# crowsonkb/k-diffusion

Measured on AMD Instinct MI355X. Metric: images/sec, 256x256 image_transformer_v2, 50-step DPM++2M (whole job), higher is better.
Workload: dtype f32

## Files before the change

include/kdiff_hip.h:

```cpp
#ifndef KDIFF_HIP_H
#define KDIFF_HIP_H

#ifdef __cplusplus
extern "C" {
#endif

#define KD_OK 0
#define KD_EINVAL (-1)
#define KD_ELAUNCH (-2)

int kd_version(void);
const char* kd_last_error(void);
int kd_set_option(const char* name, int value);
int kd_get_option(const char* name, int dflt);

enum { KD_A_PLAIN = 0, KD_A_MERGE2x2 = 1, KD_A_PATCH_NCHW = 2 };
enum { KD_PREC_EXACT = 0, KD_PREC_SPLIT3 = 1,
       KD_PREC_BF16 = 2  };
enum { KD_EPI_STORE = 0, KD_EPI_RESIDUAL = 1, KD_EPI_GEGLU = 2, KD_EPI_SPLIT_LERP = 3, KD_EPI_UNPATCH_NCHW = 4,
       KD_EPI_QKV = 5  };

typedef struct {
  int M, N, K;
  int a_mode, epi;
// ... 21 lines not shown
  int qkv_packed;
  const float* rope_pos;
  const float* rope_freq;
  int a_split, c_split;
  const void* A_lo;
  void* C_lo;
  int per_row;
} KdGemm;

int kd_gemm_f32(const KdGemm* desc, void* stream);

int kd_gemm_bf16(const KdGemm* desc, void* stream);
long long kd_packed_weight_bytes_bf16(int N, int K, int geglu);
int kd_pack_weight_bf16(const float* W, void* out, int N, int K, int geglu, void* stream);

typedef struct KdFfn {
  const void* x;
  void* out;
  const float* scale;
  int scale_stride, rows_per_sample;
  float eps;
  const void* Wp_up;
  const void* Wp_down;
  int M, K, d_ff;
  const void* attn;
  const void* Wp_out;
} KdFfn;
int kd_ffn_bf16_supported(int M, int K, int d_ff);
int kd_ffn_bf16(const KdFfn* desc, void* stream);
int kd_ffn_f32_supported(int M, int K, int d_ff);
int kd_ffn_f32(const KdFfn* desc, void* stream);
int kd_attn_ffn_f32_supported(int batch, int H, int W, int nh, int ks, int K, int d_ff);
int kd_attn_ffn_f32(const float* qkv, const KdFfn* desc, int batch, int H, int W, int nh, int ks, void* stream);

long long kd_packed_weight_bytes(int N, int K, int geglu);
int kd_pack_weight_bf16x3(const float* W, void* out, int N, int K, int geglu, void* stream);

int kd_norm_split_f32(const float* x, const float* scale, int scale_stride, int rows_per_sample, void* hi, void* lo, int M, int K,
                      float eps, void* stream);

int kd_rmsnorm_f32(const float* x, const float* scale, float* y, int rows, int d, float eps, void* stream);

int kd_fourier_sigma_f32(const float* sigma, const float* weight, float* ff, int batch, int half, void* stream);
int kd_fourier_f32(const float* in, const float* weight, float* ff, int batch, int in_dim, int half, void* stream);
int kd_cond_sum_f32(float* out, const float* a, const float* b, int b_rows, const float* emb,
                    const long long* ids, const float* c, int batch, int d, void* stream);

int kd_qk_prep_f32(float* qkv, const float* scale_h, const float* cos_t, const float* sin_t,
                   int batch, int tokens_per_sample, int nh, float eps, void* stream);

int kd_attn_global_f32(const float* qkv, float* out, int batch, int T, int nh,
                       int prep, const float* scale_h, const float* cos_t, const float* sin_t, float eps,
                       int precision, void* stream);

int kd_attn_window_f32(const float* qkv, float* out, int batch, int H, int W, int nh, int ws, int shift,
                       int prep, const float* scale_h, const float* cos_t, const float* sin_t, float eps,
                       int precision, void* stream);

int kd_attn_na2d_f32(const float* qkv, float* out, int batch, int H, int W, int nh, int ks,
                     int prep, const float* scale_h, const float* cos_t, const float* sin_t, float eps,
                     int precision, void* stream);

int kd_attn_global_bf16(const void* qkv, void* out, int batch, int T, int nh, void* stream);
int kd_attn_window_bf16(const void* qkv, void* out, int batch, int H, int W, int nh, int ws, int shift, void* stream);
int kd_attn_na2d_bf16(const void* qkv, void* out, int batch, int H, int W, int nh, int ks, void* stream);

// ... 142 lines not shown

int kd_pack_conv_x3(const float* w, void* out, int c_out, int c_in, int ks, void* stream);
int kd_conv2d_x3(const float* x, int ldx, const void* wp, const float* bias, const float* res, int ldr, float* y, int ldy, int batch, int H, int W,
                 int c_in, int c_out, int ks, void* stream);
int kd_conv2d_x3_stacked(const float* x, int ldx, const void* wp, const float* bias, const float* res, int ldr, float* y, int ldy, int batch, int H,
                         int W, int c_in, int c_out, int ks, int bias_batch, void* stream);
int kd_groupnorm_stats_f32(const float* x, int ldx, float* stats, int batch, int hw, int chan, int groups, float eps, void* stream);
int kd_groupnorm_stats_jvp_f32(const float* x, int ldx, const float* x_dot, int ldxd, float* stats, float* jstats, int batch, int hw, int chan,
                               int groups, float eps, void* stream);
int kd_adagn_apply_f32(const float* x, int ldx, const float* stats, const float* wb, int wb_stride, float* y, int ldy, int batch, int hw, int chan,
                       int groups, int gelu, void* stream);
int kd_adagn_apply_jvp_f32(const float* x, int ldx, const float* x_dot, int ldxd, const float* stats, const float* jstats, const float* wb,
                           int wb_stride, float* y, int ldy, float* y_dot, int ldyd, int batch, int hw, int chan, int groups, int gelu, void* stream);
int kd_down2_f32(const float* x, int ldx, float* y, int ldy, int batch, int H, int W, int chan, void* stream);
int kd_up2_f32(const float* x, int ldx, float* y, int ldy, int batch, int H, int W, int chan, void* stream);
int kd_unet_in_f32(const float* img, const float* w, const float* bias, const float* sigma, float sigma_data, float* y, int ldy, int batch, int hw,
                   int c_img, int chan, void* stream);
int kd_unet_out_f32(const float* x, int ldx, const float* w, const float* bias, const float* img, const float* sigma, float sigma_data, float* out,
                    int batch, int hw, int c_img, int chan, void* stream);
int kd_cond_mlp_f32(const float* x, const float* w, const float* bias, const float* add, float* y, int rows, int n_out, int k_in, int gelu,
                    void* stream);

int kd_to_uint8(const float* x, unsigned char* y, long long n, void* stream);

int kd_prof_enable(int on);
int kd_prof_count(void);
int kd_prof_get(int i, char* name, int name_cap, float* ms, double* flops, double* bytes);
int kd_prof_reset(void);
int kd_prof_clock_buffer(void* dev_ptr);

enum { KD_OP_GEMM_F32 = 0, KD_OP_GEMM_BF16 = 1, KD_OP_FFN_F32 = 2, KD_OP_FFN_BF16 = 3,
       KD_OP_ATTN_GLOBAL_F32 = 4, KD_OP_ATTN_WINDOW_F32 = 5, KD_OP_ATTN_NA2D_F32 = 6,
       KD_OP_ATTN_GLOBAL_BF16 = 7, KD_OP_ATTN_WINDOW_BF16 = 8, KD_OP_ATTN_NA2D_BF16 = 9, KD_OP_NORM_SPLIT_F32 = 10,
       KD_OP_ATTN_BLOCK_BF16 = 11, KD_OP_PROJ_BLOCK_BF16 = 12, KD_OP_GEMM_MX8 = 13, KD_OP_ATTN_FFN_F32 = 14 };
typedef struct {
  int op;
  float f;
  const void* p[5];
  int i[8];
} KdCall;
int kd_run_list(const KdCall* calls, int n, void* stream, int* failed);

#ifdef __cplusplus
}
#endif
#endif
```

k-diffusion_amd/_native.py:

```python
import ctypes as C
import os

_HERE = os.path.dirname(os.path.abspath(__file__))
LIB_PATH = os.environ.get("KDIFF_HIP_LIB") or os.path.join(_HERE, "csrc", "libkdiff_hip.so")

A_PLAIN, A_MERGE2x2, A_PATCH_NCHW = 0, 1, 2
EPI_STORE, EPI_RESIDUAL, EPI_GEGLU, EPI_SPLIT_LERP, EPI_UNPATCH_NCHW, EPI_QKV = 0, 1, 2, 3, 4, 5
PREC_EXACT, PREC_SPLIT3, PREC_BF16 = 0, 1, 2
PC_ONE, PC_SKIP, PC_OUT, PC_IN = 0, 1, 2, 3
WG_PLAIN, WG_MERGE2x2, WG_PATCH_NCHW = 0, 1, 2
LW_KARRAS, LW_SOFT_MIN_SNR, LW_SNR, LW_GIVEN = 0, 1, 2, 3
PREC_FP8 = 3
_MODES = {"exact": PREC_EXACT, "split3": PREC_SPLIT3, "bf16": PREC_BF16, "fp8": PREC_FP8}


def default_precision():
    mode = os.environ.get("KDIFF_GEMM", "split3").lower()
    if mode not in _MODES:
        raise ValueError(f"KDIFF_GEMM={mode!r}: expected one of {sorted(_MODES)}")
    return _MODES[mode]


def kernel_precision():
    p = default_precision()
# ... 39 lines not shown

class KdMtTensor(C.Structure):
    _fields_ = [("p", C.c_void_p), ("g", C.c_void_p), ("m", C.c_void_p), ("v", C.c_void_p), ("ema", C.c_void_p),
                ("n", C.c_longlong), ("group", C.c_int), ("reserved", C.c_int)]


class KdAdamGroup(C.Structure):
    _fields_ = [("lr", C.c_double), ("wd", C.c_double), ("beta1", C.c_double), ("beta2", C.c_double), ("eps", C.c_double),
                ("bc1", C.c_double), ("bc2", C.c_double)]


MT_CHUNK = 8192
(DENSITY_LOGNORMAL, DENSITY_LOGLOGISTIC, DENSITY_LOGUNIFORM, DENSITY_V_DIFFUSION, DENSITY_COSINE_INTERPOLATED,
 DENSITY_SPLIT_LOGNORMAL) = range(6)

_vp, _i, _f, _ll, _d = C.c_void_p, C.c_int, C.c_float, C.c_longlong, C.c_double
_u, _ull = C.c_uint, C.c_ulonglong

SIGNATURES = {
    "kd_version": [],
    "kd_last_error": [],
    "kd_set_option": [C.c_char_p, _i],
    "kd_get_option": [C.c_char_p, _i],
    "kd_gemm_f32": [C.POINTER(KdGemm), _vp],
    "kd_gemm_bf16": [C.POINTER(KdGemm), _vp],
    "kd_packed_weight_bytes_bf16": [_i, _i, _i],
    "kd_pack_weight_bf16": [_vp, _vp, _i, _i, _i, _vp],
    "kd_ffn_bf16_supported": [_i, _i, _i],
    "kd_ffn_bf16": [_vp, _vp],
    "kd_ffn_f32_supported": [_i, _i, _i],
    "kd_ffn_f32": [_vp, _vp],
    "kd_attn_ffn_f32_supported": [_i, _i, _i, _i, _i, _i, _i],
    "kd_attn_ffn_f32": [_vp, _vp, _i, _i, _i, _i, _i, _vp],
    "kd_attn_global_bf16": [_vp, _vp, _i, _i, _i, _vp],
    "kd_attn_window_bf16": [_vp, _vp, _i, _i, _i, _i, _i, _i, _vp],
    "kd_attn_na2d_bf16": [_vp, _vp, _i, _i, _i, _i, _i, _vp],
    "kd_attn_block_bf16_supported": [_i, _i, _i],
    "kd_attn_block_bf16": [C.POINTER(KdGemm), _vp],
    "kd_proj_block_bf16_supported": [_i, _i, _i, _i],
    "kd_proj_block_bf16": [C.POINTER(KdGemm), _vp],
    "kd_packed_weight_bytes_mx8": [_i, _i, _i],
    "kd_pack_weight_mx8": [_vp, _vp, _i, _i, _i, _vp],
    "kd_gemm_mx8_supported": [_i, _i, _i, _i, _i],
    "kd_gemm_mx8": [C.POINTER(KdGemm), _vp],
    "kd_packed_weight_bytes": [_i, _i, _i],
    "kd_pack_weight_bf16x3": [_vp, _vp, _i, _i, _i, _vp],
    "kd_rmsnorm_f32": [_vp, _vp, _vp, _i, _i, _f, _vp],
    "kd_fourier_sigma_f32": [_vp, _vp, _vp, _i, _i, _vp],
    "kd_fourier_f32": [_vp, _vp, _vp, _i, _i, _i, _vp],
    "kd_cond_sum_f32": [_vp, _vp, _vp, _i, _vp, _vp, _vp, _i, _i, _vp],
    "kd_qk_prep_f32": [_vp, _vp, _vp, _vp, _i, _i, _i, _f, _vp],
    "kd_attn_global_f32": [_vp, _vp, _i, _i, _i, _i, _vp, _vp, _vp, _f, _i, _vp],
    "kd_attn_window_f32": [_vp, _vp, _i, _i, _i, _i, _i, _i, _i, _vp, _vp, _vp, _f, _i, _vp],
    "kd_attn_na2d_f32": [_vp, _vp, _i, _i, _i, _i, _i, _i, _vp, _vp, _vp, _f, _i, _vp],
    "kd_sampler_step_f32": [_i, _vp, _vp, _vp, _vp, _vp, _f, _f, _f, _f, _ll, _vp],
    "kd_precond_in_f32": [_vp, _vp, _vp, _f, _i, _ll, _vp],
    "kd_precond_out_f32": [_vp, _vp, _vp, _vp, _f, _i, _ll, _vp],
    "kd_rows_affine_f32": [_vp, _vp, _vp, _vp, _vp, _i, _ll, _vp],
    "kd_sigma_to_t_f32": [_vp, _vp, _vp, _i, _i, _i, _vp],
    "kd_t_to_sigma_f32": [_vp, _vp, _vp, _i, _i, _vp],
    "kd_dpm_eps_f32": [_vp, _vp, _vp, _f, _ll, _vp],
    "kd_dpm_combine_f32": [_vp, _vp, _vp, _vp, _f, _f, _ll, _vp],
    "kd_dpm_error_partials": [],
    "kd_dpm_error_f32": [_vp, _vp, _vp, _f, _f, _ll, _vp, _vp],
    "kd_brownian_f32": [_vp, _vp, _i, _ll, _d, _d, _d, _d, _f, _i, _vp],
    "kd_brownian_cached_f32": [_vp, _vp, _vp, _i, _i, _vp, _i, _ll, _d, _d, _d, _d, _f, _i, _vp],
# ... 42 lines not shown
    "kd_row_rrms_f32": [_vp, _vp, _ll, _i, _f, _vp],
    "kd_colsum_f32": [_vp, _vp, _vp, _vp, _ll, _i, _ll, _i, _vp, _vp, _vp],
    "kd_attn_scale_grad_f32": [_vp, _vp, _i, _i, _vp, _vp],
    "kd_class_emb_grad_f32": [_vp, _vp, _i, _i, _i, _i, _vp, _vp],
    "kd_loss_prep_f32": [_vp, _vp, _vp, _f, _vp, _vp, _i, _ll, _vp],
    "kd_loss_f32": [_vp, _vp, _vp, _vp, _f, _i, _vp, _vp, _i, _ll, _vp],
    "kd_loss_vjp_f32": [_vp, _vp, _vp, _vp, _f, _i, _vp, _vp, _vp, _i, _ll, _vp],
    "kd_mmd_poly_f32": [_vp, _ll, _ll, _vp, _ll, _ll, _i, _i, _i, _vp, _f, _i, _vp, _vp],
    "kd_poly_kernel_f32": [_vp, _ll, _ll, _vp, _ll, _ll, _i, _i, _i, _vp, _vp],
    "kd_mmd_mats_f32": [_vp, _vp, _vp, _ll, _ll, _i, _vp, _vp, _vp],
    "kd_jacobi_sweep_f64": [_vp, _vp, _i, _i, _d, _vp, _vp, _vp],
    "kd_sym_lower_f64": [_vp, _i, _vp, _vp, _i, _i, _d, _vp],
    "kd_row_sqrt_norm_f64": [_vp, _ll, _i, _vp, _vp],
    "kd_gemm_tn_f64": [_vp, _vp, _vp, _i, _i, _i, _i, _vp, _vp, _vp],
    "kd_center_f32": [_vp, _vp, _ll, _i, _vp, _vp, _vp],
    "kd_transpose_f64": [_vp, _vp, _i, _i, _vp],
    "kd_sqrtm_vjp_div_f64": [_vp, _vp, _i, _i, _vp, _vp],
    "kd_f32_to_f64": [_vp, _vp, _ll, _vp],
    "kd_fid_finish_f32": [_vp, _vp, _vp, _vp, _vp, _i, _vp, _vp],
    "kd_mt_sqnorm_f32": [_vp, _vp, _i, _f, _vp, _vp, _vp],
    "kd_mt_adamw_ema_f32": [_vp, _vp, _i, _vp, _i, _vp, _d, _i, _i, _vp],
    "kd_mt_lerp_f32": [_vp, _vp, _i, _d, _vp],
    "kd_sigma_density_f32": [_i, _vp, _i, _vp, _vp, _i, _ll, _i, _i, _i, _vp, _vp],
    "kd_prof_enable": [_i],
    "kd_prof_count": [],
    "kd_prof_get": [_i, C.c_char_p, _i, C.POINTER(C.c_float), C.POINTER(C.c_double), C.POINTER(C.c_double)],
    "kd_prof_reset": [],
    "kd_prof_clock_buffer": [_vp],
    "kd_run_list": [C.POINTER(KdCall), _i, _vp, C.POINTER(C.c_int)],
}

RUN_LIST_OPS = {"kd_gemm_f32": 0, "kd_gemm_bf16": 1, "kd_ffn_f32": 2, "kd_ffn_bf16": 3, "kd_attn_global_f32": 4, "kd_attn_window_f32": 5,
                "kd_attn_na2d_f32": 6, "kd_attn_global_bf16": 7, "kd_attn_window_bf16": 8, "kd_attn_na2d_bf16": 9, "kd_norm_split_f32": 10,
                "kd_attn_block_bf16": 11, "kd_proj_block_bf16": 12, "kd_gemm_mx8": 13, "kd_attn_ffn_f32": 14}


def encode_call(call, name, args):
    op = RUN_LIST_OPS.get(name)
    if op is None:
        return False
    kinds = SIGNATURES[name][:-1]
    if len(kinds) != len(args):
        raise ValueError(f"{name}: {len(args)} arguments for {len(kinds)} parameters")
    call.op = op
    n_p = n_i = 0
    for kind, a in zip(kinds, args):
        if kind is _i:
            call.i[n_i] = int(a)
            n_i += 1
        elif kind is _f:
            call.f = a.value if isinstance(a, C.c_float) else float(a)
        else:
            if hasattr(a, "bind_call"):
                a.bind_call(call, n_p)
                v = a.scale
            elif isinstance(a, C.Structure):
                v = C.addressof(a)
            elif isinstance(a, C.c_void_p):
                v = a.value
            else:
                v = a
            call.p[n_p] = v
            n_p += 1
    return True

_lib = None

# ... 81 lines not shown
```

k-diffusion_amd/csrc/attn_ffn_x3.hip:

```cpp
#include "attn_x3_core.h"
#include "ffn_x3h_core.h"

namespace kd {
namespace x3 {

extern unsigned long long* g_clk;

constexpr int AF_KS = 7;
constexpr int AF_LDS_FFN = 4 * STG + 4 * 1024 + 4 * 2048;
constexpr int AF_LDS = x3a::NaGeo<AF_KS>::LDS > AF_LDS_FFN ? x3a::NaGeo<AF_KS>::LDS : AF_LDS_FFN;
static_assert(AF_LDS <= 80 * 1024, "two workgroups per CU");

struct PanelTile {
  static constexpr bool ATT_LDS = true;
  int tok0, W;
  __device__ __forceinline__ int row(int i) const { return tok0 + (4 * (i >> 6) + ((i & 31) >> 3)) * W + 8 * ((i >> 5) & 1) + (i & 7); }
};

__global__ __launch_bounds__(256, 2) void attn_ffn_x3h_kernel(const x3a::NArgs a, const FArgs3 p) {
  using namespace x3a;
  extern __shared__ __attribute__((aligned(16))) char smem[];
  const int tid = threadIdx.x;
  const auto warm = code_warm_begin<28 * 1024>((int)blockIdx.x < a.warm && tid < 64);
  (void)wg_stamp_begin(a.clk);
  const int tiles_x = a.W / NA_TW, tiles_y = a.H / NA_TH;
  int r = KD_XCD_CHUNK();
  const int tx = r % tiles_x; r /= tiles_x;
  const int ty = r % tiles_y, b = r / tiles_y;
  auto fresh = [&]() { int t = tid; asm volatile("" : "+v"(t)); return t; };

  f32x4 on[2][2][4];
  static_for<2>([&](auto head_) {
    constexpr int head = decltype(head_)::value;
    na2d_x3_tile<AF_KS>(smem, a, fresh(), b, head, ty, tx, [&]() { if constexpr (head == 0) code_warm_end(warm); },
                        [&](bool, int, float l, const f32x16 (&O)[2]) {
      const float inv = 1.0f / l;
#pragma unroll
      for (int e = 0; e < 2; ++e)
#pragma unroll
        for (int g = 0; g < 4; ++g) on[head][e][g] = f32x4(f32x4{O[e][4 * g], O[e][4 * g + 1], O[e][4 * g + 2], O[e][4 * g + 3]} * inv);
    });
    KD_BARRIER();
  });

  const int tid_b = fresh();
  {
    const int lane = tid_b & 63, wid = __builtin_amdgcn_readfirstlane(tid_b >> 6), l31 = lane & 31, h2 = lane >> 5;
    char* rowp = smem + wid * STG + l31 * 512;
#pragma unroll
    for (int head = 0; head < 2; ++head)
#pragma unroll
      for (int e = 0; e < 2; ++e)
#pragma unroll
        for (int g = 0; g < 4; ++g)
          *reinterpret_cast<f32x4*>(rowp + (((16 * head + 8 * e + 2 * g + h2) ^ (l31 & 15)) << 4)) = on[head][e][g];
  }
  asm volatile("s_waitcnt lgkmcnt(0)\n\t; kd_phase_b" ::: "memory");

  ffn_x3h_body<true>(p, smem, tid_b, PanelTile{(b * a.H + ty * NA_TH) * a.W + tx * NA_TW, a.W}, []() {});
  wg_stamp_end(wg_stamp_again(a.clk));
}

}
}

using namespace kd;

extern "C" int kd_attn_ffn_f32_supported(int batch, int H, int W, int nh, int ks, int K, int d_ff) {
  if (!opt(KD_OPT_attn_ffn_x3) || !opt(KD_OPT_attn_x3) || !opt(KD_OPT_ffn_x3)) return 0;
  if (ks != x3::AF_KS || nh != 2 || K != 128 || d_ff <= 0 || (d_ff & 63)) return 0;
  if (batch <= 0 || H <= 0 || W <= 0 || H % x3a::NA_TH || W % x3a::NA_TW) return 0;
  return kd_ffn_f32_supported(batch * H * W, K, d_ff);
}

extern "C" int kd_attn_ffn_f32(const float* qkv, const KdFfn* dp, int batch, int H, int W, int nh, int ks, void* stream) {
  if (!qkv || !dp) return fail(KD_EINVAL, "kd_attn_ffn_f32: null qkv / descriptor");
  const KdFfn& d = *dp;
  if (!d.x || !d.out || !d.scale || !d.Wp_up || !d.Wp_down || !d.Wp_out) return fail(KD_EINVAL, "kd_attn_ffn_f32: null x / out / scale / Wp_up / Wp_down / Wp_out");
  if (ks != x3::AF_KS || nh != 2 || d.K != 128 || d.d_ff <= 0 || (d.d_ff & 63) || batch <= 0 || H <= 0 || W <= 0 || H % x3a::NA_TH || W % x3a::NA_TW)
    return fail(KD_EINVAL, "kd_attn_ffn_f32: kernel size 7, 2 heads of 64, K = 128, d_ff a multiple of 64, token grid a multiple of 8 x 16 (ks=%d nh=%d K=%d d_ff=%d H=%d W=%d)",
                ks, nh, d.K, d.d_ff, H, W);
  if ((long long)batch * H * W != d.M || d.rows_per_sample != H * W || (d.scale_stride & 3))
    return fail(KD_EINVAL, "kd_attn_ffn_f32: M = batch H W, rows_per_sample = H W, scale_stride %% 4 == 0");
  x3a::NArgs a{qkv, nullptr, batch, H, W, nh, code_warm(), x3::g_clk};
  x3::FArgs3 f{};
  f.X = reinterpret_cast<const float*>(d.x); f.Y = reinterpret_cast<float*>(d.out);
  f.Wu = reinterpret_cast<const char*>(d.Wp_up); f.Wd = reinterpret_cast<const char*>(d.Wp_down);
  f.scale = d.scale; f.scale_stride = d.scale_stride; f.rows_per_sample = d.rows_per_sample; f.eps = d.eps;
  f.M = d.M; f.d_ff = d.d_ff; f.n_tiles = d.d_ff / 64;
  f.warm = 0;
  f.clk = x3::g_clk;
  f.Wo = reinterpret_cast<const char*>(d.Wp_out);
  const double M = d.M, K = d.K;
  const double flops = 4.0 * M * nh * x3a::DH * ks * ks + 2.0 * M * 3.0 * d.d_ff * K + 2.0 * M * K * K;
  const double bytes = 16.0 * M * nh * x3a::DH + 4.0 * (3.0 * M * K + 3.0 * d.d_ff * K + K * K) - 8.0 * M * K;
  const ProfName nm("attn_ffn_x3", "attn_ffn_x3 %dx%d nh=%d K=%d d_ff=%d", H, W, nh, d.K, d.d_ff);
  LaunchScope prof(nm, flops, bytes, (hipStream_t)stream);
  launch<x3::attn_ffn_x3h_kernel>(dim3((unsigned)(d.M / 128)), dim3(256), x3::AF_LDS, (hipStream_t)stream, a, f);
  return check_launch("kd_attn_ffn_f32");
}

KD_TEXT_PAD(attn_ffn_x3)
```

k-diffusion_amd/csrc/common.cpp:

```cpp
#include "kd_common.h"
#include <atomic>
#include <climits>
#include <mutex>

namespace kd {

static thread_local char g_err[512] = "";
char* err_buf() { return g_err; }

int fail(int code, const char* fmt, ...) {
  va_list ap;
  va_start(ap, fmt);
  vsnprintf(g_err, sizeof(g_err), fmt, ap);
  va_end(ap);
  return code;
}

static std::atomic<bool> g_prof{false};
static std::mutex g_rec_mutex;
static std::vector<ProfRec> g_recs;

bool prof_on() { return g_prof.load(std::memory_order_relaxed); }

static unsigned g_gen = 0;
// ... 96 lines not shown
  std::lock_guard<std::mutex> lock(g_rec_mutex);
  for (auto& r : g_recs) { (void)hipEventDestroy(r.e0); (void)hipEventDestroy(r.e1); }
  g_recs.clear();
  ++g_gen;
  return KD_OK;
}

extern "C" int kd_run_list(const KdCall* calls, int n, void* stream, int* failed) {
  if (!calls || n < 0) return kd::fail(KD_EINVAL, "kd_run_list: null list");
  for (int k = 0; k < n; ++k) {
    const KdCall& c = calls[k];
    const int* i = c.i;
    int rc;
    switch (c.op) {
      case KD_OP_GEMM_F32: rc = kd_gemm_f32(static_cast<const KdGemm*>(c.p[0]), stream); break;
      case KD_OP_GEMM_BF16: rc = kd_gemm_bf16(static_cast<const KdGemm*>(c.p[0]), stream); break;
      case KD_OP_FFN_F32: rc = kd_ffn_f32(static_cast<const KdFfn*>(c.p[0]), stream); break;
      case KD_OP_FFN_BF16: rc = kd_ffn_bf16(static_cast<const KdFfn*>(c.p[0]), stream); break;
      case KD_OP_ATTN_GLOBAL_F32:
        rc = kd_attn_global_f32(static_cast<const float*>(c.p[0]), static_cast<float*>(const_cast<void*>(c.p[1])), i[0], i[1], i[2], i[3], static_cast<const float*>(c.p[2]),
                                static_cast<const float*>(c.p[3]), static_cast<const float*>(c.p[4]), c.f, i[4], stream);
        break;
      case KD_OP_ATTN_WINDOW_F32:
        rc = kd_attn_window_f32(static_cast<const float*>(c.p[0]), static_cast<float*>(const_cast<void*>(c.p[1])), i[0], i[1], i[2], i[3], i[4], i[5], i[6],
                                static_cast<const float*>(c.p[2]), static_cast<const float*>(c.p[3]), static_cast<const float*>(c.p[4]), c.f, i[7], stream);
        break;
      case KD_OP_ATTN_NA2D_F32:
        rc = kd_attn_na2d_f32(static_cast<const float*>(c.p[0]), static_cast<float*>(const_cast<void*>(c.p[1])), i[0], i[1], i[2], i[3], i[4], i[5],
                              static_cast<const float*>(c.p[2]), static_cast<const float*>(c.p[3]), static_cast<const float*>(c.p[4]), c.f, i[6], stream);
        break;
      case KD_OP_ATTN_GLOBAL_BF16: rc = kd_attn_global_bf16(c.p[0], const_cast<void*>(c.p[1]), i[0], i[1], i[2], stream); break;
      case KD_OP_ATTN_WINDOW_BF16: rc = kd_attn_window_bf16(c.p[0], const_cast<void*>(c.p[1]), i[0], i[1], i[2], i[3], i[4], i[5], stream); break;
      case KD_OP_ATTN_NA2D_BF16: rc = kd_attn_na2d_bf16(c.p[0], const_cast<void*>(c.p[1]), i[0], i[1], i[2], i[3], i[4], stream); break;
      case KD_OP_NORM_SPLIT_F32:
        rc = kd_norm_split_f32(static_cast<const float*>(c.p[0]), static_cast<const float*>(c.p[1]), i[0], i[1], const_cast<void*>(c.p[2]), const_cast<void*>(c.p[3]), i[2], i[3],
                               c.f, stream);
        break;
      case KD_OP_ATTN_BLOCK_BF16:
        rc = kd_attn_block_bf16(static_cast<const KdGemm*>(c.p[0]), stream);
        break;
      case KD_OP_PROJ_BLOCK_BF16: rc = kd_proj_block_bf16(static_cast<const KdGemm*>(c.p[0]), stream); break;
      case KD_OP_GEMM_MX8: rc = kd_gemm_mx8(static_cast<const KdGemm*>(c.p[0]), stream); break;
      case KD_OP_ATTN_FFN_F32: rc = kd_attn_ffn_f32(static_cast<const float*>(c.p[0]), static_cast<const KdFfn*>(c.p[1]), i[0], i[1], i[2], i[3], i[4], stream); break;
      default: rc = kd::fail(KD_EINVAL, "kd_run_list: entry %d names no entry point (op %d)", k, c.op);
    }
    if (rc != KD_OK) {
      if (failed) *failed = k;
      return rc;
    }
  }
  return KD_OK;
}
```

k-diffusion_amd/csrc/ffn_x3h_core.h:

```cpp
#pragma once
#include "x3_common.h"

namespace kd {
namespace x3 {

struct FArgs3 {
  const float* X; float* Y;
  const char* Wu; const char* Wd;
  const float* scale; int scale_stride, rows_per_sample; float eps;
  int M, d_ff, n_tiles;
  int warm;
  unsigned long long* clk;
  const float* Att; const char* Wo;
};

template <int IDX>
__device__ __forceinline__ f32x4 areg_read4() {
  f32x4 v;
  asm volatile("v_accvgpr_read_b32 %0, a[%c4]\n\tv_accvgpr_read_b32 %1, a[%c5]\n\tv_accvgpr_read_b32 %2, a[%c6]\n\tv_accvgpr_read_b32 %3, a[%c7]"
               : "=v"(v[0]), "=v"(v[1]), "=v"(v[2]), "=v"(v[3]) : "i"(IDX), "i"(IDX + 1), "i"(IDX + 2), "i"(IDX + 3));
  return v;
}

template <int IDX>
__device__ __forceinline__ void mfma_acc_ag_lo(const bf16x8 w, const bf16x8 h) {
  asm volatile("v_mfma_f32_32x32x16_bf16 a[%c2:%c3], %0, %1, a[%c2:%c3]" :: "v"(w), "v"(h), "i"(IDX), "i"(IDX + 15) : KD_AGPR_LO128);
}
template <int IDX, int BIDX>
__device__ __forceinline__ void mfma_acc_aa_lo(const bf16x8 w) {
  asm volatile("v_mfma_f32_32x32x16_bf16 a[%c1:%c2], %0, a[%c3:%c4], a[%c1:%c2]" :: "v"(w), "i"(IDX), "i"(IDX + 15), "i"(BIDX), "i"(BIDX + 3) : KD_AGPR_LO128);
}
template <int IDX>
__device__ __forceinline__ void areg_zero16_lo() {
  static_for<16>([&](auto i_) { asm volatile("v_accvgpr_write_b32 a[%c0], 0" :: "i"(IDX + decltype(i_)::value) : KD_AGPR_LO128); });
}

struct PanelRows {
  static constexpr bool ATT_LDS = false;
  int m0;
  __device__ __forceinline__ int row(int i) const { return m0 + i; }
};

template <bool OUTP, class Panel, class WarmEnd>
__device__ __forceinline__ void ffn_x3h_body(const FArgs3& p, char* smem, int tid, const Panel& pn, WarmEnd&& warm_end) {
  constexpr int NC = 8, K = 128, NOB = 4;
  constexpr int NSTG = 4, PDIST = NSTG - 1, PB = 4, UNIT = 3;
  constexpr int AO = 64;
  constexpr int CPR = K / 4, PIECES = 32 * CPR / 64, SCL = 1024, SUB = 8192, HALF = 4096;
  const int lane = tid & 63, l31 = lane & 31, lh = lane >> 5;
  const int wid = __builtin_amdgcn_readfirstlane(tid >> 6);
  const int T2 = 2 * p.n_tiles;
  const bool probe = p.clk && blockIdx.x == (gridDim.x * 5) / 8 && tid == 0;
  if (probe) { p.clk[0] = __builtin_amdgcn_s_memtime(); p.clk[1] = __builtin_amdgcn_s_memrealtime(); }

  auto issue_rel = [&](int th, auto off_, int j) {
    constexpr int off = decltype(off_)::value, u = off % UNIT;
    const int tt = min(th + off / UNIT, T2 - 1);
    char* slot = smem + ((th * UNIT + off) % NSTG) * STG;
    const char* src;
    char* dst;
    if constexpr (u < 2) {
      src = p.Wu + ((size_t)(tt >> 1) * (NC / 2) + 2 * u + (j >> 1)) * STG + (j & 1) * IMG + (tt & 1) * HALF + wid * 1024 + lane * 16;
      dst = slot + (j >> 1) * SUB + (j & 1) * HALF + wid * 1024;
    } else {
      src = p.Wd + (size_t)tt * STG + wid * (PB * 1024) + j * 1024 + lane * 16;
      dst = slot + wid * (PB * 1024) + j * 1024;
    }
    __builtin_amdgcn_global_load_lds((const __attribute__((address_space(1))) void*)src, (__attribute__((address_space(3))) void*)dst, 16, 0, 0);
  };

  const int row = pn.row(wid * 32 + l31);
  const bool ok = row < p.M;
  const int rowc = ok ? row : p.M - 1;
  float rs = 1.f;
  f32x4 xres[OUTP ? NOB : 1][4];
  if constexpr (OUTP) {
    const float* xr = p.X + (size_t)rowc * K + 4 * lh;
// ... 286 lines not shown
        mfma_acc_ag_lo<AO + 16 * j>(w, h);
      };
      dd(I0, I0, true, false);
      __builtin_amdgcn_sched_barrier(0);
      read_dn(slot, 1, dh[1], dl[1]);
      __builtin_amdgcn_sched_barrier(0);
      dd(I0, I1, true, false); dd(I0, I2, true, false); dd(I0, I3, true, false);
      dd(I0, I0, false, true); dd(I0, I1, false, true); dd(I0, I2, false, true); dd(I0, I3, false, true);
      dd(I0, I0, false, false); dd(I0, I1, false, false); dd(I0, I2, false, false); dd(I0, I3, false, false);
      __builtin_amdgcn_sched_barrier(0);
      next_stage_in();
      dd(I1, I0, true, false);
      __builtin_amdgcn_sched_barrier(0);
      read_up(nslot, 0, uh[0], ul[0]);
      __builtin_amdgcn_sched_barrier(0);
      dd(I1, I1, true, false); dd(I1, I2, true, false);
      issue_rel(th, std::integral_constant<int, 2 + PDIST>{}, 0);
      __builtin_amdgcn_sched_barrier(0);
      dd(I1, I3, true, false); dd(I1, I0, false, true); dd(I1, I1, false, true);
      issue_rel(th, std::integral_constant<int, 2 + PDIST>{}, 1);
      __builtin_amdgcn_sched_barrier(0);
      dd(I1, I2, false, true); dd(I1, I3, false, true); dd(I1, I0, false, false);
      issue_rel(th, std::integral_constant<int, 2 + PDIST>{}, 2);
      __builtin_amdgcn_sched_barrier(0);
      dd(I1, I1, false, false); dd(I1, I2, false, false);
      issue_rel(th, std::integral_constant<int, 2 + PDIST>{}, 3);
      dd(I1, I3, false, false);
      __builtin_amdgcn_sched_barrier(0);
    }
    if (probe && th == 4) p.clk[11] = __builtin_amdgcn_s_memtime();
  }
  if (probe) p.clk[12] = __builtin_amdgcn_s_memtime();

  char* strip = smem + NSTG * STG + 4 * SCL + wid * 2048;
  float* st_row[2];
  const float* sk_row[2];
  bool st_ok[2];
#pragma unroll
  for (int it = 0; it < 2; ++it) {
    const int r = pn.row(wid * 32 + 16 * it + (lane >> 2));
    st_ok[it] = r < p.M;
    st_row[it] = p.Y + (size_t)min(r, p.M - 1) * K + 4 * (lane & 3);
    sk_row[it] = p.X + (size_t)min(r, p.M - 1) * K + 4 * (lane & 3);
  }
  f32x4 skip_all[NOB][2][2];
#pragma unroll
  for (int ob = 0; ob < NOB; ++ob)
#pragma unroll
    for (int hb = 0; hb < 2; ++hb)
#pragma unroll
      for (int it = 0; it < 2; ++it)
        skip_all[ob][hb][it] = OUTP ? f32x4{0.f, 0.f, 0.f, 0.f} : *reinterpret_cast<const f32x4*>(sk_row[it] + 32 * ob + 16 * hb);
  __builtin_amdgcn_sched_barrier(0);
  asm volatile("s_waitcnt vmcnt(0)\n\ts_nop 15\n\ts_nop 3" ::: "memory");
  static_for<NOB>([&](auto ob_) {
    constexpr int ob = decltype(ob_)::value;
    f32x4 blk[4];
    static_for<4>([&](auto g_) { blk[decltype(g_)::value] = areg_read4<AO + 16 * ob + 4 * decltype(g_)::value>(); });
#pragma unroll
    for (int hb = 0; hb < 2; ++hb) {
      const f32x4 (&skip)[2] = skip_all[ob][hb];
#pragma unroll
      for (int gg = 0; gg < 2; ++gg)
        *reinterpret_cast<f32x4*>(strip + l31 * 64 + (((2 * gg + lh) ^ ((l31 >> 2) & 1)) << 4)) = blk[2 * hb + gg];
#pragma unroll
      for (int it = 0; it < 2; ++it) {
// ... 12 lines not shown
```

k-diffusion_amd/models/image_transformer_v2.py:

```python
import ctypes as C
import os
import math
from dataclasses import dataclass
from typing import NamedTuple, Optional, Union

import torch
from torch import nn

from .. import _native as nat
from .. import ops
from .. import weights
from . import axial_rope

D_HEAD = 64
SCHEDULE_TABLE_MAX_BYTES = 1 << 30
SCHEDULES_KEPT = 4
SCHEDULE_CHAINS_KEPT = 2
DERIVED_KEPT = 1024
MAX_PLANS = 16
PLAN_SWITCHES = (("KDIFF_ATTN_BLOCK", "1"), ("KDIFF_PROJ_BLOCK", "1"), ("KDIFF_FFN_OUT", "all"), ("KDIFF_RUN_LIST", "1"), ("KDIFF_ATTN_FFN", "1"))
CLASS_IDS_KEPT = 4



@dataclass
class GlobalAttentionSpec:
    d_head: int


@dataclass
class NeighborhoodAttentionSpec:
    d_head: int
    kernel_size: int


@dataclass
class ShiftedWindowAttentionSpec:
    d_head: int
    window_size: int


@dataclass
class NoAttentionSpec:
    pass


@dataclass
class LevelSpec:
    depth: int
    width: int
    d_ff: int
    self_attn: Union[GlobalAttentionSpec, NeighborhoodAttentionSpec, ShiftedWindowAttentionSpec, NoAttentionSpec]
    dropout: float
# ... 334 lines not shown
        wide = [t * lv.width for t, lv in zip(toks, levels) if _prepass(mode, lv.width)]
        self.xn = torch.empty(max(wide), **f32) if wide else None
        norm_mods = m._ada_norm_modules()
        self.table_offsets, total = {}, 0
        for name, mod in norm_mods:
            self.table_offsets[name] = 4 * total
            total += mod.linear.weight.shape[0]
        wcat = m._packed.get("ada_norm_wcat")
        if wcat is None or wcat.device != device:
            wcat = m._packed["ada_norm_wcat"] = torch.cat([mod.linear.weight.detach() for _, mod in norm_mods], dim=0).contiguous()
        self.wcat = wcat
        self.scales = [torch.empty(B, total, **f32), torch.empty(B, total, **f32)]
        self.norm_descs = []
        self.last_buf, self.prefetched = 1, None
        self.side_stream = torch.cuda.Stream(device=device)
        self.main_entry = torch.cuda.Event()
        self.schedules, self.schedule_chains = [], {}
        self.scale_width = total
        self.step_chain = self.build_cond(B)

        L = self.launches
        self.d_patch_in = self._gemm(L, "patch_in", None, m.patch_in.proj.weight, xs[0], toks[0], levels[0].width, m.in_channels * ph * pw,
                                     a_mode=nat.A_PATCH_NCHW, grid=grids[0], patch=(ph, pw, m.in_channels))
        for st in hourglass(m):
            li = st.level
            if st.kind == "layer":
                self._add_layer(li, st.prefix, st.module, st.index)
            elif st.kind == "merge":
                self._gemm(L, f"merges.{li}", xs[li], m.merges[li].proj.weight, xs[li + 1], toks[li + 1], levels[li + 1].width,
                           4 * levels[li].width, a_mode=nat.A_MERGE2x2, grid=grids[li + 1])
            else:
                self._gemm(L, f"splits.{li}", xs[li + 1], m.splits[li].proj.weight, xs[li], toks[li + 1], 4 * levels[li].width,
                           levels[li + 1].width, epi=nat.EPI_SPLIT_LERP, residual=xs[li], fac=m.splits[li].fac, grid=grids[li + 1])
        self.d_patch_out = self._gemm(L, "patch_out", xs[0], m.patch_out.proj.weight, None, toks[0], m.out_channels * ph * pw,
                                      levels[0].width, epi=nat.EPI_UNPATCH_NCHW, norm_scale=m.out_norm.scale, scale_stride=0,
                                      rows_per_sample=grids[0][0] * grids[0][1], grid=grids[0], patch=(ph, pw, m.out_channels))
        self._encode_launches()

    def _gemm(self, launches, what, A, Wt, Cc, M, N, K, cond=False, table=None, entry=None, mx8=False, **kw):
        precision = self.cond_precision if cond else self.precision
        if table is not None:
            kw.update(scale_ptr=0, scale_stride=self.scale_width)
        d = ops.gemm(A, Wt, Cc, M=M, N=N, K=K, precision=precision, per_row=cond, mx8=mx8, launch=False, pack=self.model._packed_image, **kw)
        if table is not None:
            self.norm_descs.append((d, self.table_offsets[table]))
        launches.append(_Launch(entry or ops._gemm_entry(precision, mx8), (d,), what + ("(mx8)" if mx8 else "")))
        return d

    def _norm_split(self, launches, table, x, T, d, rps):
        ref = _ScaleRef()
        self.norm_descs.append((ref, self.table_offsets[table]))
        planes = self.xn.view(torch.bfloat16)
        hi, lo = planes[:T * d], planes[T * d:2 * T * d]
        launches.append(_Launch("kd_norm_split_f32", (_ptr(x), ref, self.scale_width, rps, _ptr(hi), _ptr(lo), T, d, 1e-6), table + " (split)"))
        return hi, lo

    def build_cond(self, rows):
        m, f32 = self.model, dict(device=self.device, dtype=torch.float32)
        mw, mdff = m.mapping_spec.width, m.mapping_spec.d_ff
        ch = _CondChain(rows, self.lib)
        L = ch.launches
        ch.c_sigma = torch.empty(rows, **f32)
        ch.class_ids = torch.zeros(rows, device=self.device, dtype=torch.int64)
        ch.aug_in = torch.zeros(rows, 9, **f32) if self.has_aug else None
        ch.map_in = torch.zeros(rows, m.mapping_cond_dim, **f32) if self.has_mapping_cond else None
        ff, temb, emb, mres, cond = (torch.empty(rows, mw, **f32) for _ in range(5))
        mh = torch.empty(rows, mdff, **f32)
        ch.keep += [ff, temb, emb, mres, cond, mh]
        L.append(_Launch("kd_fourier_sigma_f32", (_ptr(ch.c_sigma), _ptr(m.time_emb.weight), _ptr(ff), rows, mw // 2), "fourier_sigma"))
# ... 551 lines not shown
```

Measured before the change: 220.4.

## Fuse patch-out unpatch GEMM into final attention+FFN kernel tail

When the last launch of the network is the fused neighborhood-attention+FFN kernel, the output RMSNorm, patch-out projection, NCHW unpatch and optional c_skip/c_out preconditioning now run inside that kernel's epilogue, straight from its register accumulators. This drops a separate GEMM launch and the write and re-read of the final residual stream. It adds a templated tail path with its own weight staging through LDS and extra MFMA work per workgroup, which may raise register pressure. The path is restricted to split3 precision, 4x4 patches and at most 4 channels.

```diff
diff --git a/include/kdiff_hip.h b/include/kdiff_hip.h
--- a/include/kdiff_hip.h
+++ b/include/kdiff_hip.h
@@ -77,6 +77,8 @@
 int kd_ffn_f32(const KdFfn* desc, void* stream);
 int kd_attn_ffn_f32_supported(int batch, int H, int W, int nh, int ks, int K, int d_ff);
 int kd_attn_ffn_f32(const float* qkv, const KdFfn* desc, int batch, int H, int W, int nh, int ks, void* stream);
+int kd_attn_ffn_unpatch_f32_supported(int batch, int H, int W, int nh, int ks, int K, int d_ff, int ph, int pw, int chan);
+int kd_attn_ffn_unpatch_f32(const float* qkv, const KdFfn* desc, const KdGemm* tail, int batch, int H, int W, int nh, int ks, void* stream);
 
 long long kd_packed_weight_bytes(int N, int K, int geglu);
 int kd_pack_weight_bf16x3(const float* W, void* out, int N, int K, int geglu, void* stream);
@@ -285,7 +287,7 @@
 enum { KD_OP_GEMM_F32 = 0, KD_OP_GEMM_BF16 = 1, KD_OP_FFN_F32 = 2, KD_OP_FFN_BF16 = 3,
        KD_OP_ATTN_GLOBAL_F32 = 4, KD_OP_ATTN_WINDOW_F32 = 5, KD_OP_ATTN_NA2D_F32 = 6,
        KD_OP_ATTN_GLOBAL_BF16 = 7, KD_OP_ATTN_WINDOW_BF16 = 8, KD_OP_ATTN_NA2D_BF16 = 9, KD_OP_NORM_SPLIT_F32 = 10,
-       KD_OP_ATTN_BLOCK_BF16 = 11, KD_OP_PROJ_BLOCK_BF16 = 12, KD_OP_GEMM_MX8 = 13, KD_OP_ATTN_FFN_F32 = 14 };
+       KD_OP_ATTN_BLOCK_BF16 = 11, KD_OP_PROJ_BLOCK_BF16 = 12, KD_OP_GEMM_MX8 = 13, KD_OP_ATTN_FFN_F32 = 14, KD_OP_ATTN_FFN_UNPATCH_F32 = 15 };
 typedef struct {
   int op;
   float f;
diff --git a/k-diffusion_amd/_native.py b/k-diffusion_amd/_native.py
--- a/k-diffusion_amd/_native.py
+++ b/k-diffusion_amd/_native.py
@@ -95,6 +95,8 @@
     "kd_ffn_f32": [_vp, _vp],
     "kd_attn_ffn_f32_supported": [_i, _i, _i, _i, _i, _i, _i],
     "kd_attn_ffn_f32": [_vp, _vp, _i, _i, _i, _i, _i, _vp],
+    "kd_attn_ffn_unpatch_f32_supported": [_i, _i, _i, _i, _i, _i, _i, _i, _i, _i],
+    "kd_attn_ffn_unpatch_f32": [_vp, _vp, _vp, _i, _i, _i, _i, _i, _vp],
     "kd_attn_global_bf16": [_vp, _vp, _i, _i, _i, _vp],
     "kd_attn_window_bf16": [_vp, _vp, _i, _i, _i, _i, _i, _i, _vp],
     "kd_attn_na2d_bf16": [_vp, _vp, _i, _i, _i, _i, _i, _vp],
@@ -203,7 +205,8 @@
 
 RUN_LIST_OPS = {"kd_gemm_f32": 0, "kd_gemm_bf16": 1, "kd_ffn_f32": 2, "kd_ffn_bf16": 3, "kd_attn_global_f32": 4, "kd_attn_window_f32": 5,
                 "kd_attn_na2d_f32": 6, "kd_attn_global_bf16": 7, "kd_attn_window_bf16": 8, "kd_attn_na2d_bf16": 9, "kd_norm_split_f32": 10,
-                "kd_attn_block_bf16": 11, "kd_proj_block_bf16": 12, "kd_gemm_mx8": 13, "kd_attn_ffn_f32": 14}
+                "kd_attn_block_bf16": 11, "kd_proj_block_bf16": 12, "kd_gemm_mx8": 13, "kd_attn_ffn_f32": 14,
+                "kd_attn_ffn_unpatch_f32": 15}
 
 
 def encode_call(call, name, args):
diff --git a/k-diffusion_amd/csrc/attn_ffn_x3.hip b/k-diffusion_amd/csrc/attn_ffn_x3.hip
--- a/k-diffusion_amd/csrc/attn_ffn_x3.hip
+++ b/k-diffusion_amd/csrc/attn_ffn_x3.hip
@@ -17,7 +17,8 @@
   __device__ __forceinline__ int row(int i) const { return tok0 + (4 * (i >> 6) + ((i & 31) >> 3)) * W + 8 * ((i >> 5) & 1) + (i & 7); }
 };
 
-__global__ __launch_bounds__(256, 2) void attn_ffn_x3h_kernel(const x3a::NArgs a, const FArgs3 p) {
+template <class Tail>
+__global__ __launch_bounds__(256, 2) void attn_ffn_x3h_kernel(const x3a::NArgs a, const FArgs3 p, const Tail tail) {
   using namespace x3a;
   extern __shared__ __attribute__((aligned(16))) char smem[];
   const int tid = threadIdx.x;
@@ -57,7 +58,7 @@
   }
   asm volatile("s_waitcnt lgkmcnt(0)\n\t; kd_phase_b" ::: "memory");
 
-  ffn_x3h_body<true>(p, smem, tid_b, PanelTile{(b * a.H + ty * NA_TH) * a.W + tx * NA_TW, a.W}, []() {});
+  ffn_x3h_body<true>(p, smem, tid_b, PanelTile{(b * a.H + ty * NA_TH) * a.W + tx * NA_TW, a.W}, []() {}, tail);
   wg_stamp_end(wg_stamp_again(a.clk));
 }
 
@@ -73,15 +74,28 @@
   return kd_ffn_f32_supported(batch * H * W, K, d_ff);
 }
 
-extern "C" int kd_attn_ffn_f32(const float* qkv, const KdFfn* dp, int batch, int H, int W, int nh, int ks, void* stream) {
-  if (!qkv || !dp) return fail(KD_EINVAL, "kd_attn_ffn_f32: null qkv / descriptor");
+static int attn_ffn_launch(const char* who, const float* qkv, const KdFfn* dp, const KdGemm* tail, int batch, int H, int W, int nh, int ks, void* stream) {
+  if (!qkv || !dp) return fail(KD_EINVAL, "%s: null qkv / descriptor", who);
   const KdFfn& d = *dp;
-  if (!d.x || !d.out || !d.scale || !d.Wp_up || !d.Wp_down || !d.Wp_out) return fail(KD_EINVAL, "kd_attn_ffn_f32: null x / out / scale / Wp_up / Wp_down / Wp_out");
+  if (!d.x || (!tail && !d.out) || !d.scale || !d.Wp_up || !d.Wp_down || !d.Wp_out) return fail(KD_EINVAL, "%s: null x / out / scale / Wp_up / Wp_down / Wp_out", who);
   if (ks != x3::AF_KS || nh != 2 || d.K != 128 || d.d_ff <= 0 || (d.d_ff & 63) || batch <= 0 || H <= 0 || W <= 0 || H % x3a::NA_TH || W % x3a::NA_TW)
-    return fail(KD_EINVAL, "kd_attn_ffn_f32: kernel size 7, 2 heads of 64, K = 128, d_ff a multiple of 64, token grid a multiple of 8 x 16 (ks=%d nh=%d K=%d d_ff=%d H=%d W=%d)",
-                ks, nh, d.K, d.d_ff, H, W);
+    return fail(KD_EINVAL, "%s: kernel size 7, 2 heads of 64, K = 128, d_ff a multiple of 64, token grid a multiple of 8 x 16 (ks=%d nh=%d K=%d d_ff=%d H=%d W=%d)",
+                who, ks, nh, d.K, d.d_ff, H, W);
   if ((long long)batch * H * W != d.M || d.rows_per_sample != H * W || (d.scale_stride & 3))
-    return fail(KD_EINVAL, "kd_attn_ffn_f32: M = batch H W, rows_per_sample = H W, scale_stride %% 4 == 0");
+    return fail(KD_EINVAL, "%s: M = batch H W, rows_per_sample = H W, scale_stride %% 4 == 0", who);
+  x3::UnpatchTail t{};
+  if (tail) {
+    const KdGemm& g = *tail;
+    if (g.precision != KD_PREC_SPLIT3 || g.epi != KD_EPI_UNPATCH_NCHW || g.a_mode != KD_A_PLAIN || g.a_split || g.c_split || !g.norm || g.scale_stride != 0 ||
+        g.M != d.M || g.K != d.K || g.ph != 4 || g.pw != 4 || g.chan <= 0 || g.chan > 4 || g.N != 16 * g.chan || g.gh != H || g.gw != W)
+      return fail(KD_EINVAL, "%s: the tail is the split3 patch-out descriptor of the same rows: out_norm gain (scale_stride 0), 4 x 4 patches, at most 4 channels, "
+                  "patch grid = token grid (M=%d N=%d K=%d ph=%d pw=%d chan=%d gh=%d gw=%d)", who, g.M, g.N, g.K, g.ph, g.pw, g.chan, g.gh, g.gw);
+    if (!g.Wp || !g.scale || !g.C || (g.sigma && !g.R)) return fail(KD_EINVAL, "%s: tail needs Wp, scale, C (and R when sigma is given)", who);
+    t.Wp = reinterpret_cast<const char*>(g.Wp); t.scale = g.scale; t.eps = g.eps;
+    t.sigma = g.sigma; t.sigma_data = g.sigma_data;
+    t.R = reinterpret_cast<const float*>(g.R); t.C = reinterpret_cast<float*>(g.C);
+    t.gh = g.gh; t.gw = g.gw; t.chan = g.chan;
+  }
   x3a::NArgs a{qkv, nullptr, batch, H, W, nh, code_warm(), x3::g_clk};
   x3::FArgs3 f{};
   f.X = reinterpret_cast<const float*>(d.x); f.Y = reinterpret_cast<float*>(d.out);
@@ -92,12 +106,30 @@
   f.clk = x3::g_clk;
   f.Wo = reinterpret_cast<const char*>(d.Wp_out);
   const double M = d.M, K = d.K;
-  const double flops = 4.0 * M * nh * x3a::DH * ks * ks + 2.0 * M * 3.0 * d.d_ff * K + 2.0 * M * K * K;
-  const double bytes = 16.0 * M * nh * x3a::DH + 4.0 * (3.0 * M * K + 3.0 * d.d_ff * K + K * K) - 8.0 * M * K;
-  const ProfName nm("attn_ffn_x3", "attn_ffn_x3 %dx%d nh=%d K=%d d_ff=%d", H, W, nh, d.K, d.d_ff);
+  double flops = 4.0 * M * nh * x3a::DH * ks * ks + 2.0 * M * 3.0 * d.d_ff * K + 2.0 * M * K * K;
+  double bytes = 16.0 * M * nh * x3a::DH + 4.0 * (3.0 * M * K + 3.0 * d.d_ff * K + K * K) - 8.0 * M * K;
+  if (tail) {
+    flops += 2.0 * M * tail->N * K;
+    bytes += 4.0 * (M * tail->N * (tail->sigma ? 2.0 : 1.0) + (double)tail->N * K) - 4.0 * M * K;
+  }
+  const ProfName nm(tail ? "attn_ffn_unpatch_x3" : "attn_ffn_x3", tail ? "attn_ffn_unpatch_x3 %dx%d nh=%d K=%d d_ff=%d" : "attn_ffn_x3 %dx%d nh=%d K=%d d_ff=%d", H, W, nh, d.K, d.d_ff);
   LaunchScope prof(nm, flops, bytes, (hipStream_t)stream);
-  launch<x3::attn_ffn_x3h_kernel>(dim3((unsigned)(d.M / 128)), dim3(256), x3::AF_LDS, (hipStream_t)stream, a, f);
-  return check_launch("kd_attn_ffn_f32");
+  if (tail) launch<x3::attn_ffn_x3h_kernel<x3::UnpatchTail>>(dim3((unsigned)(d.M / 128)), dim3(256), x3::AF_LDS, (hipStream_t)stream, a, f, t);
+  else launch<x3::attn_ffn_x3h_kernel<x3::NoTail>>(dim3((unsigned)(d.M / 128)), dim3(256), x3::AF_LDS, (hipStream_t)stream, a, f, x3::NoTail{});
+  return check_launch(who);
+}
+
+extern "C" int kd_attn_ffn_f32(const float* qkv, const KdFfn* dp, int batch, int H, int W, int nh, int ks, void* stream) {
+  return attn_ffn_launch("kd_attn_ffn_f32", qkv, dp, nullptr, batch, H, W, nh, ks, stream);
+}
+
+extern "C" int kd_attn_ffn_unpatch_f32_supported(int batch, int H, int W, int nh, int ks, int K, int d_ff, int ph, int pw, int chan) {
+  return ph == 4 && pw == 4 && chan > 0 && chan <= 4 && kd_attn_ffn_f32_supported(batch, H, W, nh, ks, K, d_ff);
+}
+
+extern "C" int kd_attn_ffn_unpatch_f32(const float* qkv, const KdFfn* dp, const KdGemm* tail, int batch, int H, int W, int nh, int ks, void* stream) {
+  if (!tail) return fail(KD_EINVAL, "kd_attn_ffn_unpatch_f32: null patch-out descriptor");
+  return attn_ffn_launch("kd_attn_ffn_unpatch_f32", qkv, dp, tail, batch, H, W, nh, ks, stream);
 }
 
 KD_TEXT_PAD(attn_ffn_x3)
diff --git a/k-diffusion_amd/csrc/common.cpp b/k-diffusion_amd/csrc/common.cpp
--- a/k-diffusion_amd/csrc/common.cpp
+++ b/k-diffusion_amd/csrc/common.cpp
@@ -152,6 +152,9 @@
       case KD_OP_ATTN_GLOBAL_BF16: rc = kd_attn_global_bf16(c.p[0], const_cast<void*>(c.p[1]), i[0], i[1], i[2], stream); break;
       case KD_OP_ATTN_WINDOW_BF16: rc = kd_attn_window_bf16(c.p[0], const_cast<void*>(c.p[1]), i[0], i[1], i[2], i[3], i[4], i[5], stream); break;
       case KD_OP_ATTN_NA2D_BF16: rc = kd_attn_na2d_bf16(c.p[0], const_cast<void*>(c.p[1]), i[0], i[1], i[2], i[3], i[4], stream); break;
+      case KD_OP_ATTN_FFN_UNPATCH_F32:
+        rc = kd_attn_ffn_unpatch_f32(static_cast<const float*>(c.p[0]), static_cast<const KdFfn*>(c.p[1]), static_cast<const KdGemm*>(c.p[2]), i[0], i[1], i[2], i[3], i[4], stream);
+        break;
       case KD_OP_NORM_SPLIT_F32:
         rc = kd_norm_split_f32(static_cast<const float*>(c.p[0]), static_cast<const float*>(c.p[1]), i[0], i[1], const_cast<void*>(c.p[2]), const_cast<void*>(c.p[3]), i[2], i[3],
                                c.f, stream);
diff --git a/k-diffusion_amd/csrc/ffn_x3h_core.h b/k-diffusion_amd/csrc/ffn_x3h_core.h
--- a/k-diffusion_amd/csrc/ffn_x3h_core.h
+++ b/k-diffusion_amd/csrc/ffn_x3h_core.h
@@ -14,6 +14,16 @@
   const float* Att; const char* Wo;
 };
 
+struct NoTail { static constexpr bool ON = false; };
+struct UnpatchTail {
+  static constexpr bool ON = true;
+  const char* Wp;
+  const float* scale; float eps;
+  const float* sigma; float sigma_data;
+  const float* R; float* C;
+  int gh, gw, chan;
+};
+
 template <int IDX>
 __device__ __forceinline__ f32x4 areg_read4() {
   f32x4 v;
@@ -41,8 +51,8 @@
   __device__ __forceinline__ int row(int i) const { return m0 + i; }
 };
 
-template <bool OUTP, class Panel, class WarmEnd>
-__device__ __forceinline__ void ffn_x3h_body(const FArgs3& p, char* smem, int tid, const Panel& pn, WarmEnd&& warm_end) {
+template <bool OUTP, class Panel, class WarmEnd, class Tail = NoTail>
+__device__ __forceinline__ void ffn_x3h_body(const FArgs3& p, char* smem, int tid, const Panel& pn, WarmEnd&& warm_end, const Tail& tail = Tail{}) {
   constexpr int NC = 8, K = 128, NOB = 4;
   constexpr int NSTG = 4, PDIST = NSTG - 1, PB = 4, UNIT = 3;
   constexpr int AO = 64;
@@ -395,6 +405,106 @@
   }
   if (probe) p.clk[12] = __builtin_amdgcn_s_memtime();
 
+  if constexpr (Tail::ON) {
+    static_assert(OUTP, "the accumulators hold x + block(x) only when they started from x");
+    asm volatile("s_waitcnt vmcnt(0)\n\ts_nop 15\n\ts_nop 3" ::: "memory");
+    KD_BARRIER();
+    {
+      const char* ssrc = reinterpret_cast<const char*>(tail.scale);
+      __builtin_amdgcn_global_load_lds((const __attribute__((address_space(1))) void*)(ssrc + (lane * 16) % (K * 4)),
+                                       (__attribute__((address_space(3))) void*)(smem + NSTG * STG + wid * SCL), 16, 0, 0);
+#pragma unroll
+      for (int q = 0; q < 4; ++q)
+#pragma unroll
+        for (int h = 0; h < 2; ++h)
+          __builtin_amdgcn_global_load_lds((const __attribute__((address_space(1))) void*)(tail.Wp + (size_t)q * STG + h * IMG + wid * 1024 + lane * 16),
+                                           (__attribute__((address_space(3))) void*)(smem + q * IMG + h * HALF + wid * 1024), 16, 0, 0);
+    }
+    wait_vm(8);
+    float rso;
+    {
+      const float* sl = reinterpret_cast<const float*>(smem + NSTG * STG + wid * SCL) + 4 * lh;
+      float ssq = 0.f;
+      static_for<NOB>([&](auto ob_) {
+        constexpr int ob = decltype(ob_)::value;
+        f32x4 v[4], sc[4];
+        static_for<4>([&](auto g_) { v[decltype(g_)::value] = areg_read4<AO + 16 * ob + 4 * decltype(g_)::value>(); });
+#pragma unroll
+        for (int g = 0; g < 4; ++g) sc[g] = *reinterpret_cast<const f32x4*>(sl + 32 * ob + 8 * g);
+#pragma unroll
+        for (int g = 0; g < 4; ++g)
+#pragma unroll
+          for (int e = 0; e < 4; ++e) ssq = fmaf(v[g][e], v[g][e], ssq);
+        static_for<2>([&](auto hc_) {
+          constexpr int hc = decltype(hc_)::value;
+          u32x4 hi, lo;
+          split8(v[2 * hc] * sc[2 * hc], v[2 * hc + 1] * sc[2 * hc + 1], hi, lo);
+          areg_write4_lo<8 * (2 * ob + hc)>(hi);
+          areg_write4_lo<8 * (2 * ob + hc) + 4>(lo);
+        });
+      });
+      ssq += __shfl_xor(ssq, 32, 64);
+      rso = rsqrtf(ssq / (float)K + tail.eps);
+    }
+    int ou0[2], ou1[2];
+#pragma unroll
+    for (int j = 0; j < 2; ++j) {
+      const int np = 32 * j + l31, q = np >> 2, py = q / tail.chan, cch = q - py * tail.chan;
+      const int n = np < 16 * tail.chan ? (py * 4 + (np & 3)) * tail.chan + cch : np;
+      ou0[j] = swz64(n, lh);
+      ou1[j] = swz64(n, 2 + lh);
+    }
+    asm volatile("s_waitcnt vmcnt(0)" ::: "memory");
+    KD_BARRIER();
+    f32x16 oacc[2];
+    static_for<4>([&](auto q_) {
+      constexpr int q = decltype(q_)::value;
+      bf16x8 wh[2][2], wl[2][2];
+#pragma unroll
+      for (int b = 0; b < 2; ++b)
+#pragma unroll
+        for (int j = 0; j < 2; ++j) {
+          const char* st = smem + q * IMG + (b ? ou1[j] : ou0[j]);
+          wh[b][j] = *reinterpret_cast<const bf16x8*>(st);
+          wl[b][j] = *reinterpret_cast<const bf16x8*>(st + HALF);
+        }
+      static_for<2>([&](auto b_) {
+        constexpr int b = decltype(b_)::value, c = 2 * q + b;
+        static_for<2>([&](auto j_) {
+          constexpr int j = decltype(j_)::value;
+          if constexpr (c == 0) mfma_ag0<8 * c>(oacc[j], wl[b][j]);
+          else mfma_ag<8 * c>(oacc[j], wl[b][j]);
+        });
+        static_for<2>([&](auto j_) { mfma_ag<8 * c + 4>(oacc[decltype(j_)::value], wh[b][decltype(j_)::value]); });
+        static_for<2>([&](auto j_) { mfma_ag<8 * c>(oacc[decltype(j_)::value], wh[b][decltype(j_)::value]); });
+      });
+    });
+    asm volatile("s_nop 15\n\ts_nop 3" : "+v"(oacc[0]), "+v"(oacc[1]));
+    {
+      const int per = tail.gh * tail.gw, bb = rowc / per, rr = rowc - bb * per, ty = rr / tail.gw, tx = rr - ty * tail.gw;
+      float c_out = 1.f, c_skip = 0.f;
+      if (tail.sigma) {
+        const float sg = tail.sigma[bb], sd = tail.sigma_data, var = sg * sg + sd * sd;
+        c_skip = sd * sd / var;
+        c_out = sg * sd / sqrtf(var);
+      }
+      const int Himg = 4 * tail.gh, Wimg = 4 * tail.gw;
+#pragma unroll
+      for (int j = 0; j < 2; ++j)
+#pragma unroll
+        for (int g = 0; g < 4; ++g) {
+          const int q = 8 * j + 2 * g + lh, py = q / tail.chan, cch = q - py * tail.chan;
+          if (q < 4 * tail.chan && ok) {
+            const size_t o = (((size_t)bb * tail.chan + cch) * Himg + 4 * ty + py) * Wimg + 4 * tx;
+            f32x4 v = f32x4{oacc[j][4 * g], oacc[j][4 * g + 1], oacc[j][4 * g + 2], oacc[j][4 * g + 3]} * (rso * c_out);
+            if (tail.sigma) v = v + *reinterpret_cast<const f32x4*>(tail.R + o) * c_skip;
+            st16(tail.C + o, v);
+          }
+        }
+    }
+    return;
+  }
+
   char* strip = smem + NSTG * STG + 4 * SCL + wid * 2048;
   float* st_row[2];
   const float* sk_row[2];
diff --git a/k-diffusion_amd/models/image_transformer_v2.py b/k-diffusion_amd/models/image_transformer_v2.py
--- a/k-diffusion_amd/models/image_transformer_v2.py
+++ b/k-diffusion_amd/models/image_transformer_v2.py
@@ -18,7 +18,8 @@
 SCHEDULE_CHAINS_KEPT = 2
 DERIVED_KEPT = 1024
 MAX_PLANS = 16
-PLAN_SWITCHES = (("KDIFF_ATTN_BLOCK", "1"), ("KDIFF_PROJ_BLOCK", "1"), ("KDIFF_FFN_OUT", "all"), ("KDIFF_RUN_LIST", "1"), ("KDIFF_ATTN_FFN", "1"))
+PLAN_SWITCHES = (("KDIFF_ATTN_BLOCK", "1"), ("KDIFF_PROJ_BLOCK", "1"), ("KDIFF_FFN_OUT", "all"), ("KDIFF_RUN_LIST", "1"), ("KDIFF_ATTN_FFN", "1"),
+                 ("KDIFF_STEP_TAIL", "1"))
 CLASS_IDS_KEPT = 4
 
 
@@ -419,9 +420,16 @@
             else:
                 self._gemm(L, f"splits.{li}", xs[li + 1], m.splits[li].proj.weight, xs[li], toks[li + 1], 4 * levels[li].width,
                            levels[li + 1].width, epi=nat.EPI_SPLIT_LERP, residual=xs[li], fac=m.splits[li].fac, grid=grids[li + 1])
-        self.d_patch_out = self._gemm(L, "patch_out", xs[0], m.patch_out.proj.weight, None, toks[0], m.out_channels * ph * pw,
-                                      levels[0].width, epi=nat.EPI_UNPATCH_NCHW, norm_scale=m.out_norm.scale, scale_stride=0,
-                                      rows_per_sample=grids[0][0] * grids[0][1], grid=grids[0], patch=(ph, pw, m.out_channels))
+        po = dict(M=toks[0], N=m.out_channels * ph * pw, K=levels[0].width, epi=nat.EPI_UNPATCH_NCHW, norm_scale=m.out_norm.scale, scale_stride=0,
+                  rows_per_sample=grids[0][0] * grids[0][1], grid=grids[0], patch=(ph, pw, m.out_channels))
+        last = L[-1] if L else None
+        if (mode == nat.PREC_SPLIT3 and switches.get("KDIFF_STEP_TAIL", "1") != "0" and last is not None and last.name == "kd_attn_ffn_f32"
+                and self.lib.kd_attn_ffn_unpatch_f32_supported(B, *grids[0], *last.args[5:7], levels[0].width, levels[0].d_ff, ph, pw, m.out_channels)):
+            self.d_patch_out = ops.gemm(None, m.patch_out.proj.weight, None, precision=precision, launch=False,
+                                        pack=lambda Wt, N, K, geglu: m._packed_image(Wt, N, K, 2), **po)
+            L[-1] = _Launch("kd_attn_ffn_unpatch_f32", (*last.args[:2], self.d_patch_out, *last.args[2:]), last.what + "+unpatch")
+        else:
+            self.d_patch_out = self._gemm(L, "patch_out", xs[0], m.patch_out.proj.weight, None, po.pop("M"), po.pop("N"), po.pop("K"), **po)
         self._encode_launches()
 
     def _gemm(self, launches, what, A, Wt, Cc, M, N, K, cond=False, table=None, entry=None, mx8=False, **kw):
```

New measurement: 221.8 (median of 6 runs). About the same (+0.6%).
